# pangsu0613/TransCAR

Hardware: AMD Instinct MI355X
Metric: nuScenes frames/sec (6-cam+radar, 900 queries): fusion decoder (Detr3DHead.forward + box decode), FPN features resident in HBM (higher is better)
Workload: dtype f32 (linear steps and attention core of the batched launches: f16x2 split operands, 3 v_mfma_f32_16x16x32_f16 products, fp32 accumulate; activations of the 32-row tiles held as two f16 planes; 4- / 8-row tiles: f32 MFMA)

## Files before the change

transcar_amd/csrc/chain.hip:

```cpp
#include <stdlib.h>
#include <string.h>

#include <type_traits>

#include "kernels.hpp"
#ifdef TC_CHAIN_STAMPS
__device__ long long g_cam_stamps[4][8];
#define CAM_STAMP(slot)                                                                        \
  do {                                                                                         \
    if (blockIdx.x == 100 && (threadIdx.x & 63) == 0)                                          \
      g_cam_stamps[(threadIdx.x >> 6) & 3][(slot)] = __builtin_amdgcn_s_memtime();             \
  } while (0)
#endif
#include "rowdev.hpp"
#define TC_ONCE_LD(p) ldg4_stream(p)
#ifdef TC_CHAIN_DUMP
__device__ float* g_chain_dump;
__device__ long long g_chain_dump_floats;
#endif

namespace tc {

namespace {

// ... 7 lines not shown

struct StepRes {
  const float* p0; const float* p1; const float* p2; const float* p3;
  float* gd; float* gt;
  int K, N, gld, gmod;
  short kind, src, src2, dst, res, act, flags, sync, rep, si;
  int src_off, src2_off;
  int pad_;
};
struct EpiRec {
  float* gd; float* gt;
  int dst_off, res_off, dst_ld, res_ld;
  int gld, act, flags, N;
  int has_bias, woff;
  int drop_site;
  int pad1;
};
struct PreRec { const float* first; int nidx; int pad; };
template <int NW> struct StepAllT { StepRes r; EpiRec e; PreRec p[NW]; };
using StepAll = StepAllT<CH_NW>;
static_assert(sizeof(StepAllT<CH_NW>) % 16 == 0 && sizeof(StepAllT<CH_NW_MAX>) % 16 == 0, "records are copied 16 bytes at a time");
template <int N, int NW = CH_NW> struct Recs { StepAllT<NW> s[N]; };

constexpr int HM_WORDS = 8;
static_assert(HM_WORDS * 8 <= LDL * 4 && (LDL * 4) % 8 == 0, "hit masks live in a row of the logit buffer");
template <int R, int NREC>
struct ChainLds {
  StepAllT<nw_of(R)> recs[NREC];
  float unit[4][R][LD2];
  float l[R][LDL];
  float box[R][12];
  float cen[R][4];
  int gate[R];
  int rowg[R];
};
static_assert(LD5 * 1 <= 2 * LD2, "the 512-wide tile must fit two units");

#ifdef TC_CHAIN_STAMPS
#define CHAIN_DBG(v) (v)
#else
#define CHAIN_DBG(v) 0
#endif

#define MFMA44(a, b, c, grp) __builtin_amdgcn_mfma_f32_4x4x1f32((a), (b), (c), 4, (grp), 0)

enum Buf : short { B_NONE = -1, B_A = 0 , B_X , B_U1, B_U2, B_U3, B_L };
enum Kind : short {
  K_END = 0, K_LOAD, K_LINEAR, K_LN, K_POSENC, K_SAMPLE, K_REFUPD, K_TOKENS, K_RADAR_ATTN, K_BOXADD, K_RADAR_GATE,
  K_NARROW,
  K_NOP,
  K_LOADG,
  K_MASKCOPY,
  K_LN_BWD,
  K_ATTN_BWD
};
enum NSpecial : short { N_LOGITS = -1, N_CODE = -2, N_CLS = -3 };
enum Flags : short {
  F_GATE = 1,
  F_SCALEQ = 2,
  F_WOFF = 4,
  F_LN_RELU = 8,
  F_SKIP_NONEXT = 16,
  F_WAVE1 = 32,
  F_NOT_W0 = 64,
  F_LN_XP = 128,
  F_IFHIT = 256,
  F_GPRE = 512,
  F_CMASK = 1024,
  F_CMASK_SCALE = 2048,
  F_CARRY = 4096,
  F_NOT_LAYER0 = 8192,
  F_PRESYNC = 16384
};
enum GSel : short {
  G_NONE = -1, G_HS = 0, G_QK, G_VT, G_INITREF, G_ATTN_O, G_XIN, G_POS, G_CLS, G_KV0, G_KV1, G_KV2,
  G_QF, G_RFEAT, G_COUNT
};

struct StepDesc {
  short kind, wp, wp2, K, N, src, src2, dst, res, act, flags, gsel, gtsel, sync;
};
constexpr StepDesc PROG_DECODER_T[] = {
    {K_LOAD, 0, 0, 0, 0, B_NONE, B_NONE, B_U1, B_NONE, 0, 0, G_ATTN_O, G_NONE, 0},
    {K_LOAD, 0, 0, 0, 0, B_NONE, B_NONE, B_X, B_NONE, 0, 0, G_XIN, G_NONE, 1},
    {K_LINEAR, 1, -1, 256, 256, B_U1, B_NONE, B_U2, B_X, 0, 0, G_NONE, G_NONE, 1},
    {K_LN, 2, -1, 0, 0, B_U2, B_NONE, B_X, B_U1, 0, F_LN_XP, G_NONE, G_NONE, 1},
    {K_LINEAR, 3, -1, 256, N_LOGITS, B_U1, B_NONE, B_L, B_NONE, 0, 0, G_NONE, G_NONE, 0},
    {K_POSENC, 5, 6, 0, 0, B_NONE, B_NONE, B_U2, B_NONE, 0, F_NOT_W0, G_NONE, G_NONE, 1},
    {K_SAMPLE, 0, 0, 0, 0, B_L, B_NONE, B_U3, B_NONE, 0, 0, G_NONE, G_NONE, 1},
    {K_LINEAR, 7, -1, 256, 256, B_U2, B_NONE, B_U1, B_NONE, 0, 0, G_NONE, G_NONE, 1},
    {K_LINEAR, 4, -1, 256, 256, B_U3, B_NONE, B_U2, B_X, 0, 0, G_NONE, G_NONE, 1},
    {K_LN, 9, 8, 0, 0, B_U2, B_U1, B_X, B_NONE, 0, 0, G_NONE, G_NONE, 1},
    {K_LINEAR, 10, -1, 256, 512, B_X, B_NONE, B_A, B_NONE, 1, 0, G_NONE, G_NONE, 1},
    {K_LINEAR, 11, -1, 512, 256, B_A, B_NONE, B_U3, B_X, 0, 0, G_NONE, G_NONE, 1},
    {K_LN, 12, -1, 0, 0, B_U3, B_NONE, B_X, B_U1, 0, F_LN_XP, G_HS, G_NONE, 1},
    {K_LINEAR, 13, -1, 256, 256, B_X, B_NONE, B_U2, B_NONE, 1, 0, G_NONE, G_NONE, 0},
    {K_LINEAR, 16, -1, 256, 512, B_U1, B_NONE, B_NONE, B_NONE, 0, F_SCALEQ | F_SKIP_NONEXT, G_QK, G_NONE, 0},
    {K_LINEAR, 16, -1, 256, 256, B_X, B_NONE, B_NONE, B_NONE, 0, F_WOFF | F_SKIP_NONEXT, G_NONE, G_VT, 1},
    {K_LINEAR, 14, -1, 256, 256, B_U2, B_NONE, B_U3, B_NONE, 1, 0, G_NONE, G_NONE, 0},
    {K_NARROW, 15, -1, 256, N_CODE, B_U3, B_U1, B_L, B_NONE, 0, F_PRESYNC, G_NONE, G_NONE, 1},
    {K_REFUPD, 0, 0, 0, 0, B_L, B_NONE, B_NONE, B_NONE, 0, 0, G_NONE, G_NONE, 0},
    {K_END, 0, 0, 0, 0, 0, 0, 0, 0, 0, 0, 0, 0, 0}};
constexpr StepDesc PROG_DECODER_L0_T[] = {
    {K_LOAD, 0, 0, 0, 0, B_NONE, B_NONE, B_U1, B_NONE, 0, 0, G_ATTN_O, G_NONE, 0},
    {K_LOAD, 0, 0, 0, 0, B_NONE, B_NONE, B_U2, B_NONE, 0, 0, G_KV1, G_NONE, 0},
    {K_LOAD, 0, 0, 0, 0, B_NONE, B_NONE, B_X, B_NONE, 0, 0, G_XIN, G_NONE, 1},
    {K_LINEAR, 3, -1, 256, N_LOGITS, B_U1, B_NONE, B_L, B_NONE, 0, 0, G_NONE, G_NONE, 0},
// ... 25 lines not shown
    {K_LOAD, 0, 0, 0, 0, B_NONE, B_NONE, B_U1, B_NONE, 0, 0, G_POS, G_NONE, 0},
    {K_LOAD, 0, 0, 0, 0, B_NONE, B_NONE, B_X, B_NONE, 0, 0, G_XIN, G_NONE, 1},
    {K_LINEAR, 0, -1, 256, 3, B_U1, B_NONE, B_NONE, B_NONE, 2, 0, G_INITREF, G_NONE, 0},
    {K_LINEAR, 16, -1, 256, 512, B_X, B_U1, B_NONE, B_NONE, 0, F_SCALEQ, G_QK, G_NONE, 0},
    {K_LINEAR, 16, -1, 256, 256, B_X, B_NONE, B_NONE, B_NONE, 0, F_WOFF, G_NONE, G_VT, 0},
    {K_END, 0, 0, 0, 0, 0, 0, 0, 0, 0, 0, 0, 0, 0}};
constexpr StepDesc PROG_RADAR_ENC_T[] = {
    {K_TOKENS, 0, 0, 0, 0, B_NONE, B_NONE, B_A, B_NONE, 0, 0, G_NONE, G_NONE, 1},
    {K_POSENC, 0, 1, 0, 0, B_A, B_NONE, B_U3, B_NONE, 0, 0, G_NONE, G_NONE, 0},
    {K_LINEAR, 4, -1, 36, 64, B_A, B_NONE, B_X, B_NONE, 1, 0, G_NONE, G_NONE, 1},
    {K_LINEAR, 2, -1, 256, 256, B_U3, B_NONE, B_U1, B_NONE, 0, 0, G_NONE, G_NONE, 0},
    {K_LINEAR, 5, -1, 64, 128, B_X, B_NONE, B_U2, B_NONE, 1, 0, G_NONE, G_NONE, 1},
    {K_LINEAR, 6, -1, 128, 256, B_U2, B_NONE, B_X, B_NONE, 1, 0, G_NONE, G_NONE, 1},
    {K_LN, 3, -1, 0, 0, B_U1, B_NONE, B_U2, B_X, 0, F_LN_RELU, G_NONE, G_NONE, 1},
    {K_LINEAR, 7, -1, 256, 512, B_U2, B_NONE, B_NONE, B_NONE, 0, 0, G_KV0, G_NONE, 0},
    {K_LINEAR, 8, -1, 256, 512, B_U2, B_NONE, B_NONE, B_NONE, 0, 0, G_KV1, G_NONE, 0},
    {K_LINEAR, 9, -1, 256, 512, B_U2, B_NONE, B_NONE, B_NONE, 0, 0, G_KV2, G_NONE, 0},
    {K_END, 0, 0, 0, 0, 0, 0, 0, 0, 0, 0, 0, 0, 0}};
constexpr StepDesc PROG_RADAR_ENC_A_T[] = {
    {K_TOKENS, 0, 0, 0, 0, B_NONE, B_NONE, B_A, B_NONE, 0, 0, G_NONE, G_NONE, 1},
    {K_POSENC, 0, 1, 0, 0, B_A, B_NONE, B_U3, B_NONE, 0, 0, G_NONE, G_NONE, 0},
    {K_LINEAR, 4, -1, 36, 64, B_A, B_NONE, B_X, B_NONE, 1, 0, G_NONE, G_NONE, 1},
    {K_LINEAR, 2, -1, 256, 256, B_U3, B_NONE, B_U1, B_NONE, 0, 0, G_NONE, G_NONE, 0},
    {K_LINEAR, 5, -1, 64, 128, B_X, B_NONE, B_U2, B_NONE, 1, 0, G_NONE, G_NONE, 1},
    {K_LINEAR, 6, -1, 128, 256, B_U2, B_NONE, B_X, B_NONE, 1, 0, G_NONE, G_NONE, 1},
    {K_LN, 3, -1, 0, 0, B_U1, B_NONE, B_U2, B_X, 0, F_LN_RELU, G_RFEAT, G_NONE, 1},
    {K_LINEAR, 7, -1, 256, 512, B_U2, B_NONE, B_NONE, B_NONE, 0, 0, G_KV0, G_NONE, 0},
    {K_END, 0, 0, 0, 0, 0, 0, 0, 0, 0, 0, 0, 0, 0}};
constexpr StepDesc PROG_RADAR_ENC_B_T[] = {
    {K_LOAD, 0, 0, 0, 0, B_NONE, B_NONE, B_X, B_NONE, 0, 0, G_RFEAT, G_NONE, 1},
    {K_LINEAR, 8, -1, 256, 512, B_X, B_NONE, B_NONE, B_NONE, 0, 0, G_KV1, G_NONE, 0},
    {K_LINEAR, 9, -1, 256, 512, B_X, B_NONE, B_NONE, B_NONE, 0, 0, G_KV2, G_NONE, 0},
    {K_END, 0, 0, 0, 0, 0, 0, 0, 0, 0, 0, 0, 0, 0}};
constexpr StepDesc PROG_RADAR_LAYER_T[] = {
    {K_RADAR_GATE, 0, 0, 0, 0, B_NONE, B_NONE, B_NONE, B_NONE, 0, 0, G_NONE, G_NONE, 1},
    {K_LINEAR, 0, -1, 256, 256, B_X, B_NONE, B_U1, B_NONE, 0, F_SCALEQ | F_IFHIT, G_NONE, G_NONE, 1},
    {K_RADAR_ATTN, 0, 0, 0, 0, B_U1, B_NONE, B_U2, B_NONE, 0, F_IFHIT, G_NONE, G_NONE, 1},
    {K_LINEAR, 1, -1, 256, 256, B_U2, B_NONE, B_U3, B_X, 0, F_GATE | F_IFHIT, G_NONE, G_NONE, 1},
    {K_LN, 2, -1, 0, 0, B_U3, B_NONE, B_X, B_NONE, 0, 0, G_NONE, G_NONE, 1},
    {K_LINEAR, 3, -1, 256, 512, B_X, B_NONE, B_A, B_NONE, 1, 0, G_NONE, G_NONE, 1},
    {K_LINEAR, 4, -1, 512, 256, B_A, B_NONE, B_U3, B_X, 0, 0, G_NONE, G_NONE, 1},
    {K_LN, 5, -1, 0, 0, B_U3, B_NONE, B_X, B_NONE, 0, 0, G_NONE, G_NONE, 1},
    {K_LINEAR, 6, -1, 256, 256, B_X, B_NONE, B_U1, B_NONE, 0, 0, G_NONE, G_NONE, 0},
    {K_LINEAR, 11, -1, 256, 256, B_X, B_NONE, B_U2, B_NONE, 1, 0, G_NONE, G_NONE, 1},
    {K_LN, 7, -1, 0, 0, B_U1, B_NONE, B_U1, B_NONE, 0, F_LN_RELU, G_NONE, G_NONE, 0},
    {K_LINEAR, 12, -1, 256, 256, B_U2, B_NONE, B_U3, B_NONE, 1, 0, G_NONE, G_NONE, 1},
    {K_LINEAR, 8, -1, 256, 256, B_U1, B_NONE, B_U2, B_NONE, 0, 0, G_NONE, G_NONE, 1},
    {K_LN, 9, -1, 0, 0, B_U2, B_NONE, B_U2, B_NONE, 0, F_LN_RELU, G_NONE, G_NONE, 0},
    {K_NARROW, 13, -1, 256, N_CODE, B_U3, B_U1, B_L, B_NONE, 0, F_PRESYNC, G_NONE, G_NONE, 0},
    {K_NARROW, 10, -1, 256, N_CLS, B_U2, B_U1, B_NONE, B_NONE, 0, F_PRESYNC, G_CLS, G_NONE, 1},
    {K_BOXADD, 0, 0, 0, 0, B_L, B_NONE, B_NONE, B_NONE, 0, 0, G_NONE, G_NONE, 1},
    {K_END, 0, 0, 0, 0, 0, 0, 0, 0, 0, 0, 0, 0, 0}};

constexpr StepDesc PROG_RADAR_BWD_T[] = {
    {K_LOADG, 0, 0, 0, N_CODE, B_NONE, B_NONE, B_U1, B_NONE, 0, F_CARRY, G_NONE, G_NONE, 1},
    {K_LINEAR, 13, -1, N_CODE, 256, B_U1, B_NONE, B_U2, B_NONE, 0, F_CMASK, G_NONE, G_NONE, 1},
    {K_LINEAR, 12, -1, 256, 256, B_U2, B_NONE, B_U1, B_NONE, 0, F_CMASK, G_NONE, G_NONE, 1},
    {K_LINEAR, 11, -1, 256, 256, B_U1, B_NONE, B_U3, B_X, 0, 0, G_NONE, G_NONE, 1},
    {K_LOADG, 0, 0, 0, N_CLS, B_NONE, B_NONE, B_U1, B_NONE, 0, 0, G_NONE, G_NONE, 1},
    {K_LINEAR, 10, -1, N_CLS, 256, B_U1, B_NONE, B_U2, B_NONE, 0, 0, G_NONE, G_NONE, 1},
    {K_LN_BWD, 9, -1, 0, 0, B_U2, B_NONE, B_U1, B_X, 0, F_LN_RELU, G_NONE, G_NONE, 1},
    {K_LINEAR, 8, -1, 256, 256, B_U1, B_NONE, B_U2, B_NONE, 0, 0, G_NONE, G_NONE, 1},
    {K_LN_BWD, 7, -1, 0, 0, B_U2, B_NONE, B_U1, B_X, 0, F_LN_RELU, G_NONE, G_NONE, 1},
    {K_LINEAR, 6, -1, 256, 256, B_U1, B_NONE, B_X, B_U3, 0, 0, G_NONE, G_NONE, 1},
    {K_LN_BWD, 5, -1, 0, 0, B_X, B_NONE, B_X, B_U1, 0, 0, G_NONE, G_NONE, 1},
    {K_MASKCOPY, 0, 0, 3, 0, B_X, B_NONE, B_U3, B_NONE, 0, 0, G_NONE, G_NONE, 1},
    {K_LINEAR, 4, -1, 256, 512, B_U3, B_NONE, B_A, B_NONE, 0, F_CMASK | F_CMASK_SCALE, G_NONE, G_NONE, 1},
    {K_LINEAR, 3, -1, 512, 256, B_A, B_NONE, B_U3, B_X, 0, 0, G_NONE, G_NONE, 1},
    {K_LN_BWD, 2, -1, 0, 0, B_U3, B_NONE, B_X, B_U1, 0, 0, G_NONE, G_NONE, 1},
    {K_MASKCOPY, 0, 0, 1, 0, B_X, B_NONE, B_U1, B_NONE, 0, F_GATE, G_NONE, G_NONE, 1},
    {K_LINEAR, 1, -1, 256, 256, B_U1, B_NONE, B_U2, B_NONE, 0, 0, G_NONE, G_NONE, 1},
    {K_ATTN_BWD, 0, 0, 0, 0, B_U2, B_NONE, B_U1, B_NONE, 0, 0, G_NONE, G_NONE, 1},
    {K_LINEAR, 0, -1, 256, 256, B_U1, B_NONE, B_X, B_X, 0, F_NOT_LAYER0, G_NONE, G_NONE, 1},
    {K_END, 0, 0, 0, 0, 0, 0, 0, 0, 0, 0, 0, 0, 0}};
enum DSel : short { D_NONE = -1, D_DBOX = 0, D_DT1, D_DT0, D_DC2, D_DC0, D_DFF, D_DH, D_DPROJ, D_DQP, D_DCLS, D_COUNT };
constexpr short BWD_STORE[19] = {D_DBOX, D_DT1, D_DT0, D_NONE, D_DCLS, D_NONE, D_DC2, D_NONE, D_DC0, D_NONE, D_NONE, D_DFF,
                                 D_DH, D_NONE, D_NONE, D_DPROJ, D_NONE, D_DQP, D_NONE};
enum Program : int { PROG_PROLOGUE = 0, PROG_DECODER, PROG_RADAR_ENC, PROG_RADAR, PROG_RADAR_ENC_A, PROG_RADAR_ENC_B,
                     PROG_RADAR_TRAIN, PROG_RADAR_ENC_TRAIN, PROG_RADAR_BWD };
constexpr bool prog_is_radar(int p) { return p == PROG_RADAR || p == PROG_RADAR_TRAIN; }
constexpr bool prog_is_enc_full(int p) { return p == PROG_RADAR_ENC || p == PROG_RADAR_ENC_TRAIN; }
enum TSel : short { T_NONE = -1, T_QP = 0, T_AO, T_X1, T_X2, T_H, T_FF, T_X3, T_C0, T_C1, T_C2, T_C3, T_T0, T_T1, T_TREG,
                    E_U0, E_U1, E_U2, E_POS, E_F0, E_F1, E_F2, E_MEM, T_COUNT };
constexpr short RADAR_TAPE[17] = {T_NONE, T_QP, T_AO, T_X1, T_X2, T_H, T_FF, T_X3, T_C0, T_T0, T_C1, T_T1, T_C2, T_C3,
                                  T_TREG, T_NONE, T_NONE};
constexpr short ENC_TAPE[10] = {T_NONE, E_U1, E_F0, E_U2, E_F1, E_F2, E_MEM, T_NONE, T_NONE, T_NONE};
constexpr short ENC_TAPE2[10] = {T_NONE, E_U0, T_NONE, T_NONE, T_NONE, T_NONE, E_POS, T_NONE, T_NONE, T_NONE};
constexpr short BWD_TAPE[19] = {T_NONE, T_T1, T_T0, T_NONE, T_NONE, T_NONE, T_C2, T_NONE, T_C0, T_NONE, T_X2, T_NONE,
                                T_H, T_NONE, T_X1, T_NONE, T_NONE, T_NONE, T_NONE};
constexpr short BWD_TAPE2[19] = {T_NONE, T_NONE, T_NONE, T_NONE, T_NONE, T_NONE, T_C3, T_NONE, T_C1, T_NONE, T_FF, T_NONE,
                                 T_NONE, T_NONE, T_NONE, T_NONE, T_NONE, T_NONE, T_NONE};

constexpr int MAX_PAIRS = 48;
constexpr int RADAR_PAIRS = 14;

struct ChainDev {
  int program, M, Q, code, ncls, nlogits, has_next, nlayers;
  int total, early_n;
  float* g[G_COUNT]; int g_ld[G_COUNT]; int g_mod[G_COUNT];
  float qscale; int qpad;
  DropK drop;
  int dbg;
  int tile_rows;
  int matrix_path;
  int last_cls_only;
  const float* ref_in; int ref_mod; float* ref_out; float* box_m;
// ... 1133 lines not shown
          if (row < R) act_st4<PL>(dst + row * LD2, 4 * lane, early_v[j][ri]);
        }
      }
    }
  }
#pragma unroll
  for (int t = 0; t < REC_TRIPS; ++t) {
    const int i = threadIdx.x + t * NT;
    if (i < REC16) reinterpret_cast<int4*>(&S.recs[0])[i] = rec_v[t];
  }
  START_STAMP(43);

  if (prog_is_radar(PROG)) {
    auto row_of = [&](int row) {
      const int pos = min(m0 + row, M - 1);
      return k.row_perm != nullptr ? k.row_perm[pos] : pos;
    };
    if (threadIdx.x < R) S.rowg[threadIdx.x] = row_of(threadIdx.x);
    for (int row = wave; row < R; row += NW) {
      const int grow = row_of(row);
      act_st4<PL>(&S.unit[0][row][0], 4 * lane, TC_ONCE_LD(k.g[G_QF] + (size_t)grow * 256 + 4 * lane));
    }
    {
      const int row = threadIdx.x >> 4, j = threadIdx.x & 15;
      if (row < R) {
        const int grow = row_of(row);
        if (j < k.code) S.box[row][j] = k.box_in[(size_t)grow * k.code + j];
        if (j >= 12 && j < 15) {
          const int c = j - 12;
          if (k.cen_from_box) {
            S.cen[row][c] = k.box_in[(size_t)grow * k.code + (c == 2 ? 4 : c)];
          } else {
            const float r = k.ref_last[(size_t)grow * 3 + c];
            const float* pc = k.cam.pc;
            S.cen[row][c] = c < 2 ? __fadd_rn(__fmul_rn(r, pc[3 + c] - pc[c]), pc[c]) : r;
          }
        }
      }
    }
  }
  if constexpr (PROG == PROG_RADAR_BWD) {
    for (int i = threadIdx.x; i < R * LD2; i += NT) (&S.unit[0][0][0])[i] = 0.0f;
    if (threadIdx.x < R * 12) (&S.box[0][0])[threadIdx.x] = 0.0f;
    if (threadIdx.x < R) S.gate[threadIdx.x] = 0;
  }
  __syncthreads();

  START_STAMP(46);
#ifdef TC_CHAIN_STAMPS
  int stamp_i = 0;
  STEP_STAMP();
#endif

  auto do_ln = [&](const StepRes& r) {
    constexpr int NR = R / NW;
    const float* a = buf_ptr(S, r.src); const int lda = buf_ld(r.src);
    const float* c = buf_ptr(S, r.src2); const int ldc = buf_ld(r.src2);
    const bool xp = (r.flags & F_LN_XP) != 0;
    const float* dd = xp ? nullptr : buf_ptr(S, r.res);
    float* dst2 = xp ? buf_ptr(S, r.res) : nullptr;
    float* dst = buf_ptr(S, r.dst);
    float* gdst = r.gd;
    float4 gg, bb;
    if (CHAIN_DBG(k.dbg) & (1 << 17)) {
      gg = make_float4(1.f, 1.f, 1.f, 1.f); bb = make_float4(0.f, 0.f, 0.f, 0.f);
    } else {
      gg = ld4(r.p0 + 4 * lane); bb = ld4(r.p1 + 4 * lane);
    }
    float4 v[NR], pos4[NR];
#pragma unroll
    for (int i = 0; i < NR; ++i) {
      const int row = wave + NW * i;
      pos4[i] = make_float4(0.f, 0.f, 0.f, 0.f);
      if (xp && !(CHAIN_DBG(k.dbg) & (1 << 18))) {
        int prow = min(m0 + row, M - 1);
        if (k.g_mod[G_POS] > 0) prow = prow % k.g_mod[G_POS];
        pos4[i] = ld4(k.g[G_POS] + (size_t)prow * k.g_ld[G_POS] + 4 * lane);
      }
      v[i] = act_ld4<PL>(a + row * lda, 4 * lane);
    }
    if (c != nullptr) {
      const float4 g2 = ld4(r.p2 + 4 * lane), b2 = ld4(r.p3 + 4 * lane);
      float4 cv[NR];
#pragma unroll
      for (int i = 0; i < NR; ++i) cv[i] = act_ld4<PL>(c + (wave + NW * i) * ldc, 4 * lane);
      ln_rows<NR>(cv, g2, b2);
#pragma unroll
      for (int i = 0; i < NR; ++i) v[i] = add4(v[i], relu4(cv[i]));
    }
    ln_rows<NR>(v, gg, bb);
#pragma unroll
    for (int i = 0; i < NR; ++i) {
      const int row = wave + NW * i;
      if (r.flags & F_LN_RELU) v[i] = relu4(v[i]);
      if constexpr (PROG == PROG_RADAR_ENC_TRAIN) {
        if (r.gt != nullptr && m0 + row < M) st4(r.gt + (size_t)(m0 + row) * 256 + 4 * lane, v[i]);
      }
      if (dd != nullptr) v[i] = add4(v[i], act_ld4<PL>(dd + row * LD2, 4 * lane));
      act_st4<PL>(dst + row * LD2, 4 * lane, v[i]);
      if (xp) act_st4<PL>(dst2 + row * LD2, 4 * lane, add4(v[i], pos4[i]));
      if (gdst != nullptr && m0 + row < M) st4(gdst + (size_t)(m0 + row) * 256 + 4 * lane, v[i]);
    }
  };
  auto lin_spec = [&](const StepRes& r) {
    LinSpec s;
    s.K = r.K; s.N = r.N;
    s.W = r.p0; s.bias = r.p1;
    const float* lbase = reinterpret_cast<const float*>(smem_raw);
    s.src = lbase + r.src_off; s.src_ld = buf_ld(r.src);
// ... 23 lines not shown
    s.act = e.act;
    s.scale = (e.flags & F_SCALEQ) ? k.qscale : 1.0f; s.scale_cols = (e.flags & F_SCALEQ) ? 256 : 0;
    s.gdst = e.gd; s.gdst_ld = e.gld;
    s.gt = (e.flags & F_CMASK) ? nullptr : e.gt; s.gt_ld = k.qpad; s.gt_rpb = k.Q;
    s.cmask = (e.flags & F_CMASK) ? e.gt : nullptr;
    s.cscale = (e.flags & F_CMASK_SCALE) ? k.rdrop.scale : 1.0f;
    s.m0 = m0; s.M = M;
    s.woff = e.woff;
    s.dbg = 0;
    s.sub_on = 0;
    s.drop_site = 0; s.drop_seed = 0; s.drop_thr = 0; s.drop_scale = 1.0f; s.drop_stride = 0; s.drop_q = 0;
    s.rowg = (prog_is_radar(PROG) && k.row_perm != nullptr) ? &S.rowg[0] : nullptr;
    s.gpre = (e.flags & F_GPRE) ? 1 : 0;
    s.dst_pl = PL && e.dst_ld != LDL; s.res_pl = PL && e.res_ld != LDL;
    s.range_flag = MM == 1 ? k.range_status : nullptr;
    if (DROP) {
      if constexpr (PROG == PROG_RADAR_TRAIN) {
        s.drop_site = e.drop_site; s.drop_seed = k.rdrop.seed; s.drop_thr = k.rdrop.thr; s.drop_scale = k.rdrop.scale;
      } else {
        s.drop_site = e.drop_site; s.drop_seed = k.drop.seed; s.drop_thr = k.drop.thr; s.drop_scale = k.drop.scale;
        s.drop_stride = k.drop.seed_stride; s.drop_q = (int)k.drop.rows_per_sample;
      }
    }
    return s;
  };

  auto tile_has_hit = [&]() {
    int any = 0;
#pragma unroll
    for (int i = 0; i < R; ++i) any |= S.gate[i];
    return __builtin_amdgcn_readfirstlane(any) > 0;
  };

#ifdef TC_CHAIN_DUMP
  auto dump_step = [&](int step, int dst_id) {
    if constexpr (PROG == PROG_RADAR) {
      __syncthreads();
      float* out = g_chain_dump;
      const float* src = buf_ptr(S, dst_id);
      if (out != nullptr && src != nullptr && dst_id != B_L && (long long)(step + 1) * M * 256 <= g_chain_dump_floats) {
        const int ld = buf_ld(dst_id);
        for (int row = wave; row < R; row += NW)
          if (m0 + row < M)
            st4(out + ((size_t)step * M + S.rowg[row]) * 256 + 4 * lane, *reinterpret_cast<const float4*>(src + row * ld + 4 * lane));
      }
      __syncthreads();
    }
  };
#define DUMP_STEP(step, dst) dump_step((step), (dst))
#else
#define DUMP_STEP(step, dst) do {} while (0)
#endif
  int idx = (CHAIN_DBG(k.dbg) & 16) ? total : early_n;
#ifdef TC_CHAIN_STAMPS
  for (int j = 0; j < 2 * early_n; ++j) STEP_STAMP();
#endif
#pragma unroll 1
  while (idx < total) {
    const int kind = ufirst(S.recs[idx].r.kind);
    if (kind == K_LINEAR || kind == K_LN || kind == K_NOP) {
      WBuf w0;
      int pre_idx = -1;
#ifdef TC_CHAIN_STAMPS
      int ln_rep = 0;
#endif
#pragma unroll 1
      for (;;) {
        const StepRes r = load_uniform<StepRes>(S.recs[idx].r);
        const int kd = r.kind;
        bool skip = false;
        if constexpr (PROG == PROG_RADAR) {
          if (kd == K_LINEAR && (r.flags & F_IFHIT)) skip = !tile_has_hit();
        }
        if (skip) {
          if (r.res != B_NONE && r.dst != B_NONE) {
            const float* rs = buf_ptr(S, r.res); const int rld = buf_ld(r.res);
            float* dd = buf_ptr(S, r.dst);
            for (int row = wave; row < R; row += NW)
              *reinterpret_cast<float4*>(dd + row * LD2 + 4 * lane) = *reinterpret_cast<const float4*>(rs + row * rld + 4 * lane);
          }
        } else if (kd == K_LINEAR) {
          LinSpec s = lin_spec(r);
#ifdef TC_CHAIN_STAMPS
          s.sub_on = (r.si == g_sub_step && r.rep == 0);
          SUB_STAMP(0);
#endif
          if (((wave - s.woff) & (NW - 1)) < (R == 32 ? (s.N + 31) >> 5 : (s.N + 63) >> 6)) {
            const PreRec pr = load_uniform<PreRec>(S.recs[idx].p[wave]);
            const bool have = linear_step<R, DROP, PROG == PROG_PROLOGUE, MM, MP>(s, w0, pre_idx == idx, pr.first, epi_spec, idx);
            pre_idx = have ? pr.nidx : -1;
          }
        } else if (kd == K_LN) {
          if (!(CHAIN_DBG(k.dbg) & 4)) do_ln(r);
#ifdef TC_CHAIN_STAMPS
          if (ln_rep < ((k.dbg >> 19) & 3)) { ++ln_rep; continue; }
          ln_rep = 0;
#endif
        } else if (kd != K_NOP) {
          break;
        }
        STEP_STAMP();
        if (r.sync && !(CHAIN_DBG(k.dbg) & 2)) __syncthreads();
        STEP_STAMP();
        DUMP_STEP(idx, r.dst);
        if (++idx >= total) break;
      }
      continue;
    }
    const StepRes r = load_uniform<StepRes>(S.recs[idx].r);
    const int rep = r.rep;
    switch (kind) {
      case K_LOAD: { if constexpr (PROG == PROG_DECODER || PROG == PROG_PROLOGUE || PROG == PROG_RADAR_ENC_B) {
        constexpr int MAXL = 3, RW = (R + NW - 1) / NW;
        int n = 1;
        while (n < MAXL && idx + n < total && ufirst(S.recs[idx + n].r.kind) == K_LOAD) ++n;
        float4 v[MAXL][RW];
        float* dsts[MAXL];
        int any_sync = 0;
#pragma unroll
        for (int j = 0; j < MAXL; ++j) {
          if (j < n) {
            const StepRes rj = load_uniform<StepRes>(S.recs[idx + j].r);
            const float* gsrc = rj.gd;
            const int ld = rj.gld, mod = rj.gmod;
            dsts[j] = buf_ptr(S, rj.dst);
            any_sync |= rj.sync;
#pragma unroll
            for (int ri = 0; ri < RW; ++ri) {
              int grow = min(m0 + wave + ri * NW, M - 1);
              if (mod > 0) grow = grow % mod;
              v[j][ri] = TC_ONCE_LD(gsrc + (size_t)grow * ld + 4 * lane);
            }
          }
        }
#pragma unroll
        for (int j = 0; j < MAXL; ++j) {
          if (j < n) {
#pragma unroll
            for (int ri = 0; ri < RW; ++ri) {
              const int row = wave + ri * NW;
              if (row < R) act_st4<PL>(dsts[j] + row * LD2, 4 * lane, v[j][ri]);
            }
          }
        }
        for (int j = 0; j < n; ++j) { STEP_STAMP(); STEP_STAMP(); }
        if (any_sync) __syncthreads();
        idx += n;
        continue;
      }
      } break;
      case K_TOKENS: { if constexpr (prog_is_enc_full(PROG) || PROG == PROG_RADAR_ENC_A) {
        if constexpr (PL) {
          for (int i = threadIdx.x; i < R * 16; i += NT) {
            const int row = i >> 4, c4 = 4 * (i & 15);
            const int grow = min(m0 + row, M - 1);
            const float* tk = k.tokens + (size_t)grow * k.RI;
            act_st4<PL>(&S.unit[1][0][0] + row * LD5, c4,
// ... 198 lines not shown
        const int N = r.N;
        const int c = lane & 15, g = lane >> 4;
        const int rgw = wave >> 2, kq = wave & 3;
        const float* Wn = uptr(r.p0) + (size_t)min(c, N - 1) * 256 + 4 * g;
        const float* src = buf_ptr(S, r.src) + min(16 * rgw + c, R - 1) * buf_ld(r.src);
        float4 av[4], bw[4];
#pragma unroll
        for (int q = 0; q < 4; ++q) bw[q] = ld4(Wn + 16 * (4 * kq + q));
        const float bias = r.p1 != nullptr ? ldg1(uptr(r.p1) + min(c, N - 1)) : 0.0f;
        if (r.flags & F_PRESYNC) __syncthreads();
#pragma unroll
        for (int q = 0; q < 4; ++q) av[q] = act_ld4<PL>(src, 4 * g + 16 * (4 * kq + q));
        f32x4 acc = {0.f, 0.f, 0.f, 0.f};
#pragma unroll
        for (int q = 0; q < 4; ++q) {
          acc = MFMA16(av[q].x, bw[q].x, acc); acc = MFMA16(av[q].y, bw[q].y, acc);
          acc = MFMA16(av[q].z, bw[q].z, acc); acc = MFMA16(av[q].w, bw[q].w, acc);
        }
        float* part = buf_ptr(S, r.src2);
#pragma unroll
        for (int i = 0; i < 4; ++i) part[(wave * 16 + 4 * g + i) * 16 + c] = acc[i];
        __syncthreads();
        if (kq == 0 && c < N) {
          float y[4];
#pragma unroll
          for (int i = 0; i < 4; ++i) {
            const int prow = 4 * g + i;
            float v = part[(wave * 16 + prow) * 16 + c];
#pragma unroll
            for (int w = 1; w < 4; ++w) v += part[((wave + w) * 16 + prow) * 16 + c];
            y[i] = v + bias;
          }
          if (r.dst != B_NONE) {
            float* dd = buf_ptr(S, r.dst) + c;
            const int dld = buf_ld(r.dst);
#pragma unroll
            for (int i = 0; i < 4; ++i)
              if (16 * rgw + 4 * g + i < R) dd[(16 * rgw + 4 * g + i) * dld] = y[i];
          }
          if (r.gd != nullptr) {
#pragma unroll
            for (int i = 0; i < 4; ++i) {
              const int row = 16 * rgw + 4 * g + i;
              if (row < R && m0 + row < M) {
                int grow = m0 + row;
                if constexpr (prog_is_radar(PROG)) grow = S.rowg[row];
                stg1(r.gd + (size_t)grow * r.gld + c, y[i]);
              }
            }
          }
        }
      } break;
      } break;
      case K_RADAR_GATE: { if constexpr (prog_is_radar(PROG)) {
        constexpr int GW = 4;
        const bool keep = k.T <= 64 * HM_WORDS, cached = k.T <= 64 * GW;
        const int b0 = S.rowg[wave] / k.Q;
        float ty0[GW], ty1[GW];
        if (cached) {
          const float* rxy = k.tokens + (size_t)b0 * k.T * k.RI;
#pragma unroll
          for (int w = 0; w < GW; ++w) {
            const int t = min(64 * w + lane, k.T - 1);
            ty0[w] = rxy[(size_t)t * k.RI]; ty1[w] = rxy[(size_t)t * k.RI + 1];
          }
        }
        if (threadIdx.x < R) {
          const int i = threadIdx.x;
          const GateGeom::Pre pp = GateGeom::precompute(S.box[i][3], S.box[i][6], S.box[i][7], k.rmin[rep], k.rmax[rep]);
          S.box[i][10] = pp.ox; S.box[i][11] = pp.oy; S.cen[i][3] = pp.tstar;
        }
        __syncthreads();
#pragma unroll 1
        for (int row = wave; row < R; row += NW) {
          const int grow = S.rowg[row];
          const int b = grow / k.Q;
          int count = 0;
          if (cached && b == b0) {
            const GateGeom gg(S.cen[row][0], S.cen[row][1], GateGeom::Pre{S.box[row][10], S.box[row][11], S.cen[row][3]});
#pragma unroll
            for (int w = 0; w < GW; ++w) {
              if (64 * w < k.T) {
                const unsigned long long mask =
                    __ballot(64 * w + lane < k.T && gg.hit(ty0[w], ty1[w], sqnorm2(ty0[w], ty1[w])));
                count += __popcll(mask);
                if (k.T - 1 >= 64 * w && k.T - 1 < 64 * w + 64 && ((mask >> (k.T - 1 - 64 * w)) & 1ull)) count += k.pad_mult - 1;
                if (lane == 0) reinterpret_cast<unsigned long long*>(&S.l[row][0])[w] = mask;
              }
            }
          } else {
            count = radar_gate_count(S.cen[row][0], S.cen[row][1], S.box[row][3], S.box[row][6], S.box[row][7],
                                     k.rmin[rep], k.rmax[rep], k.tokens + (size_t)b * k.T * k.RI, k.RI, k.T,
                                     k.pad_mult, lane, keep ? reinterpret_cast<unsigned long long*>(&S.l[row][0]) : nullptr);
          }
          if (lane == 0) {
            S.gate[row] = count;
            if (m0 + row < M) k.hits[(size_t)rep * (k.hits_stride ? k.hits_stride : (size_t)M) + grow] = count;
          }
        }
      } break;
      } break;
      case K_RADAR_ATTN: { if constexpr (prog_is_radar(PROG)) {
        if (PROG == PROG_RADAR && (r.flags & F_IFHIT) && !tile_has_hit()) break;
#pragma unroll 1
        for (int row = wave; row < R; row += NW) {
          const int grow = S.rowg[row];
          const int b = grow / k.Q;
          float4 q4 = act_ld4<PL>(buf_ptr(S, r.src) + row * LD2, 4 * lane);
          const float* kv = (rep == 0 ? k.g[G_KV0] : rep == 1 ? k.g[G_KV1] : k.g[G_KV2]);
          int count = 0;
          const GateGeom gg(S.cen[row][0], S.cen[row][1], GateGeom::Pre{S.box[row][10], S.box[row][11], S.cen[row][3]});
          const unsigned long long* hm = k.T <= 64 * HM_WORDS ? reinterpret_cast<const unsigned long long*>(&S.l[row][0]) : nullptr;
          float4 o;
          if constexpr (PROG == PROG_RADAR_TRAIN) {
            q4.x *= k.qscale; q4.y *= k.qscale; q4.z *= k.qscale; q4.w *= k.qscale;
            DropK dk = k.rdrop;
            dk.site = 4u * (unsigned)rep;
            o = radar_attn_row_g<true>(gg, q4, k.tokens + (size_t)b * k.T * k.RI, k.RI, kv + (size_t)b * k.T * 512, 512,
                                       k.T, k.pad_mult, lane, count, dk, grow, hm);
            if (m0 + row < M) st4(r.gd + (size_t)grow * 256 + 4 * lane, o);
          } else {
            o = radar_attn_row_g(gg, q4, k.tokens + (size_t)b * k.T * k.RI, k.RI, kv + (size_t)b * k.T * 512, 512,
                                 k.T, k.pad_mult, lane, count, DropK(), 0, hm);
          }
          act_st4<PL>(buf_ptr(S, r.dst) + row * LD2, 4 * lane, o);
          if (lane == 0) S.gate[row] = count;
        }
      } break;
      } break;
      case K_LOADG: { if constexpr (PROG == PROG_RADAR_BWD) {
        const int N = r.N;
        float* dst = buf_ptr(S, r.dst);
        const float* src = uptr(r.p0);
        const bool carry = (r.flags & F_CARRY) != 0;
        for (int i = threadIdx.x; i < R * 64; i += NT) {
          const int row = i >> 6, c = i & 63;
          const int grow = min(m0 + row, M - 1);
          float v = c < N ? ldg1(src + (size_t)grow * N + c) : 0.0f;
          if (k.loss_vals != nullptr) {
            const float lv = k.loss_vals[2 * (k.nlayers - 1 - rep) + (carry ? 1 : 0)];
            if (!(fabsf(lv) <= 3.0e38f) || !(fabsf(v) <= 3.0e38f)) v = 0.0f;
          }
          if (carry && c < N) v += S.box[row][c];
          if (c < N && r.gd != nullptr && m0 + row < M) stg1(r.gd + (size_t)grow * N + c, v);
          dst[row * LD2 + c] = v;
        }
        if (carry) {
          __syncthreads();
          const int layer = k.nlayers - 1 - rep;
          if (blockIdx.x == 0 && threadIdx.x < 2 && k.loss_vals != nullptr && k.loss_out != nullptr) {
            const float lv = k.loss_vals[2 * layer + threadIdx.x];
            k.loss_out[2 * layer + threadIdx.x] = lv != lv ? 0.0f : lv;
          }
          if (threadIdx.x < R * 16) {
            const int row = threadIdx.x >> 4, c = threadIdx.x & 15;
            if (c < 12) S.box[row][c] = (c == 0 || c == 1 || c == 4) ? dst[row * LD2 + c] : 0.0f;
// ... 74 lines not shown
#pragma unroll
            for (int w = 1; w < NW; ++w) t += scratch[w * 256 + threadIdx.x];
            if (k.detp != nullptr) acc_add(*k.detp, gdst + threadIdx.x, t);
            else unsafeAtomicAdd(gdst + threadIdx.x, t);
          }
        }
      } break;
      } break;
      case K_ATTN_BWD: { if constexpr (PROG == PROG_RADAR_BWD) {
        const int layer = k.nlayers - 1 - rep;
        const float* dao = buf_ptr(S, r.src);
        float* dqb = buf_ptr(S, r.dst);
        DropK dk = k.rdrop;
        dk.site = 4u * (unsigned)layer;
        for (int row = wave; row < R; row += NW) {
          const int grow = min(m0 + row, M - 1);
          const int b = grow / k.Q;
          float4 dq = make_float4(0.f, 0.f, 0.f, 0.f);
          if (S.gate[row] > 0 && m0 + row < M) {
            const float* cxy = k.bwd_cxy[layer] + (size_t)grow * k.bwd_ldc[layer];
            const float* bx = k.bwd_box[layer] + (size_t)grow * k.code;
            float4 q4 = ld4(uptr(r.p0) + (size_t)grow * 256 + 4 * lane);
            q4.x *= k.qscale; q4.y *= k.qscale; q4.z *= k.qscale; q4.w *= k.qscale;
            const float4 o4 = ld4(uptr(r.p1) + (size_t)grow * 256 + 4 * lane);
            const float4 dO = *reinterpret_cast<const float4*>(dao + row * LD2 + 4 * lane);
            dq = radar_attn_bwd_row(cxy[0], cxy[1], bx[3], bx[6], bx[7], k.rmin[layer], k.rmax[layer], q4,
                                    k.tokens + (size_t)b * k.T * k.RI, k.RI, uptr(r.p2) + (size_t)b * k.T * 512,
                                    const_cast<float*>(uptr(r.p3)) + (size_t)b * k.T * 512, 512, k.T, k.pad_mult, dO, o4,
                                    dk, grow, lane,
                                    k.detp != nullptr ? det_shadow_of(*k.detp, uptr(r.p3) + (size_t)b * k.T * 512) : nullptr);
            dq.x *= k.qscale; dq.y *= k.qscale; dq.z *= k.qscale; dq.w *= k.qscale;
          }
          *reinterpret_cast<float4*>(dqb + row * LD2 + 4 * lane) = dq;
          if (r.gd != nullptr && m0 + row < M) st4(r.gd + (size_t)grow * 256 + 4 * lane, dq);
        }
      } break;
      } break;
      case K_BOXADD: { if constexpr (prog_is_radar(PROG)) {
        const int row = threadIdx.x >> 4, j = threadIdx.x & 15;
        if (row < R && j < k.code) {
          const int c = j == 0 ? 0 : j == 1 ? 1 : j == 4 ? 2 : -1;
          float bx = S.l[row][j];
          if (c >= 0) { bx += S.cen[row][c]; S.cen[row][c] = bx; }
          S.box[row][j] = bx;
          if (m0 + row < M) k.all_box[((size_t)rep * M + S.rowg[row]) * k.code + j] = bx;
        }
      } break;
      } break;
      default: break;
    }
    STEP_STAMP();
    if (r.sync) __syncthreads();
    STEP_STAMP();
    DUMP_STEP(idx, r.dst);
    ++idx;
  }
  WG_STAMP(1);
}

template <int R, int PROG, bool DROP = false, int MM = 0, bool PRE = false, bool MP = false>
__global__ __launch_bounds__(nw_of(R) * 64, 2) void chain_kernel(ChainDev k, Recs<rec_cap(PROG), nw_of(R)> recs) {
  chain_body<R, PROG, DROP, MM, PRE, MP>(k, recs.s, blockIdx.x);
}

template <int RA, int RB, int PROGB, int MM = 0, bool PRE = false, bool MP = false>
__global__ __launch_bounds__(nw_of(RA) * 64, 2) void chain_dual_kernel(ChainDev ka, ChainDev kb, int na,
                                                           Recs<rec_cap(PROG_DECODER), nw_of(RA)> ra,
                                                           Recs<rec_cap(PROGB), nw_of(RB)> rb) {
  static_assert(nw_of(RA) == nw_of(RB), "both programs of a launch run with the same workgroup size");
  if ((int)blockIdx.x < na) chain_body<RA, PROG_DECODER, false, MM, PRE, MP>(ka, ra.s, blockIdx.x);
  else chain_body<RB, PROGB, false, MM>(kb, rb.s, (int)blockIdx.x - na);
}

template <int R, int PROG>
int lds_off(int id) {
  using Lds = ChainLds<R, rec_cap(PROG)>;
  const int unit0 = (int)(offsetof(Lds, unit) / 4), ustride = R * LD2;
  switch (id) {
    case B_A: return unit0 + ustride;
    case B_X: return unit0;
    case B_U1: return unit0 + ustride;
    case B_U2: return unit0 + 2 * ustride;
    case B_U3: return unit0 + 3 * ustride;
    case B_L: return (int)(offsetof(Lds, l) / 4);
    default: return -1;
  }
}
template <int R, int PROG>
constexpr size_t chain_lds_bytes() { return sizeof(ChainLds<R, rec_cap(PROG)>); }
inline int buf_ld_h(int id) { return id == B_A ? LD5 : id == B_L ? LDL : LD2; }

template <int R, int PROG, int MM = 0>
void resolve_program(ChainK& k, StepAllT<nw_of(R)>* out) {
  constexpr int NW = nw_of(R);
  const StepDesc* table = prog_table(PROG);
  int nsteps = table_steps(PROG);
  if (PROG == PROG_DECODER && k.l0_seq != 0) {
    table = k.l0_seq == 1 ? PROG_DECODER_L0_T : PROG_DECODER_L0GEN_T;
    nsteps = (int)((k.l0_seq == 1 ? sizeof(PROG_DECODER_L0_T) : sizeof(PROG_DECODER_L0GEN_T)) / sizeof(StepDesc)) - 1;
  }
  const int nrep = (prog_is_radar(PROG) || PROG == PROG_RADAR_BWD) ? k.nlayers : 1;
  const int total = nsteps * nrep;
  memset(out, 0, sizeof(StepAllT<NW>) * rec_cap(PROG));
  for (int idx = 0; idx < total; ++idx) {
    const int rep = idx / nsteps, si = idx - rep * nsteps;
    const int layer = PROG == PROG_RADAR_BWD ? k.nlayers - 1 - rep : rep;
    const int pair0 = (prog_is_radar(PROG) || PROG == PROG_RADAR_BWD) ? layer * RADAR_PAIRS : 0;
    const StepDesc d = table[si];
    StepRes& r = out[idx].r;
    r.K = d.K; r.N = d.N;
    r.kind = d.kind; r.src = d.src; r.src2 = d.src2; r.dst = d.dst; r.res = d.res; r.act = d.act;
    r.flags = d.flags; r.sync = d.sync; r.rep = (short)rep; r.si = (short)si;
    if ((d.flags & F_SKIP_NONEXT) && !k.has_next) r.kind = K_NOP;
    if (PROG == PROG_DECODER && !k.refine &&
        (d.kind == K_REFUPD || ((d.kind == K_LINEAR || d.kind == K_NARROW) && d.wp >= 13 && d.wp <= 15)))
      r.kind = K_NOP;
    if (PROG == PROG_RADAR && k.last_cls_only && rep + 1 < nrep && d.wp >= 6 && d.wp <= 10 &&
        (d.kind == K_LINEAR || d.kind == K_LN || d.kind == K_NARROW))
      r.kind = K_NOP;
    if (d.gsel != G_NONE) { r.gd = k.g[d.gsel]; r.gld = k.g_ld[d.gsel]; r.gmod = k.g_mod[d.gsel]; }
    if (d.gtsel != G_NONE) r.gt = k.g[d.gtsel];
    bool taped = false;
    if (PROG == PROG_RADAR_TRAIN) {
      if (d.flags & F_SCALEQ) r.flags = (short)(r.flags & ~F_SCALEQ);
      r.flags = (short)(r.flags & ~F_IFHIT);
      if (d.kind == K_LINEAR && d.wp == 4) r.flags = (short)(r.flags | F_GPRE);
      const short ts = RADAR_TAPE[si];
      if (ts != T_NONE && r.gd == nullptr) { r.gd = k.tape[ts] + (size_t)rep * k.tape_stride; r.gld = 256; taped = true; }
    }
    if (PROG == PROG_RADAR_BWD) {
      if ((d.flags & F_NOT_LAYER0) && layer == 0) r.kind = K_NOP;
      const short ds = BWD_STORE[si], ts = BWD_TAPE[si], ts2 = BWD_TAPE2[si];
      if (ds != D_NONE && k.dy[ds] != nullptr) { r.gd = k.dy[ds] + (size_t)layer * k.dy_stride; taped = true; }
      const float* t1 = ts != T_NONE ? k.tape[ts] + (size_t)layer * k.tape_stride : nullptr;
      const float* t2 = ts2 != T_NONE ? k.tape[ts2] + (size_t)layer * k.tape_stride : nullptr;
      if (d.kind == K_LINEAR && (d.flags & F_CMASK)) r.gt = const_cast<float*>(t1);
      if (d.kind == K_LN_BWD) {
        const tc_linear n = k.pairs[pair0 + d.wp], gn = k.gpairs[pair0 + d.wp];
        r.p0 = n.w; r.p1 = t1; r.p2 = t2; r.gt = const_cast<float*>(gn.w); r.p3 = gn.b;
      }
      if (d.kind == K_LOADG) {
        r.N = d.N == N_CODE ? k.code : k.ncls;
        r.p0 = (d.N == N_CODE ? k.d_box : k.d_cls) + (size_t)layer * k.M * r.N;
      }
      if (d.kind == K_MASKCOPY) r.K = d.K;
      if (d.kind == K_ATTN_BWD) {
        r.p0 = k.tape[T_QP] + (size_t)layer * k.tape_stride; r.p1 = k.tape[T_AO] + (size_t)layer * k.tape_stride;
        r.p2 = k.g[G_KV0 + layer]; r.p3 = k.dkv[layer];
      }
    }
    if (PROG == PROG_RADAR_ENC_TRAIN) {
      const short ts = ENC_TAPE[si], ts2 = ENC_TAPE2[si];
      if (ts != T_NONE && r.gd == nullptr) { r.gd = k.tape[ts]; r.gld = 256; taped = true; }
      if (ts2 != T_NONE) r.gt = k.tape[ts2];
    }
    if (PROG == PROG_DECODER && d.N == N_LOGITS && generic_xattn(k)) r.dst = B_U3;
    if (d.kind == K_LINEAR) {
      const tc_linear pr = k.pairs[pair0 + d.wp];
      r.K = d.K == 36 ? k.RI : d.K == N_CODE ? k.code : d.K == N_CLS ? k.ncls : d.K;
      r.N = d.N == N_LOGITS ? k.nlogits : d.N == N_CODE ? k.code : d.N == N_CLS ? k.ncls : d.N;
      const int woff = (d.flags & F_WOFF) ? 512 : 0;
      r.p0 = pr.w + (size_t)woff * ((r.K + 63) & ~63);
      if (R >= 16) r.p0 += (MM == 1 ? 2 : 1) * k.w16_delta;
      r.p1 = pr.b ? pr.b + woff : nullptr;
      if (PROG == PROG_RADAR_BWD) r.p1 = nullptr;
      if (d.gsel == G_CLS) r.gd += (size_t)rep * k.M * k.ncls;
      if (taped) r.gld = r.N;
    } else if (d.kind == K_NARROW) {
      const tc_linear pr = k.pairs[pair0 + d.wp];
      r.N = d.N == N_CODE ? k.code : d.N == N_CLS ? k.ncls : d.N;
      r.p0 = pr.w; r.p1 = pr.b;
      if (d.gsel == G_CLS) r.gd += (size_t)rep * k.M * k.ncls;
      if (taped) r.gld = r.N;
    } else if (d.kind == K_LN || d.kind == K_POSENC) {
      const tc_linear n = k.pairs[pair0 + d.wp];
      r.p0 = n.w; r.p1 = n.b;
      if (d.kind == K_POSENC || d.src2 != B_NONE) {
        const tc_linear n2 = k.pairs[pair0 + d.wp2];
        r.p2 = n2.w; r.p3 = n2.b;
      }
    }
    r.src_off = lds_off<R, PROG>(r.src); r.src2_off = lds_off<R, PROG>(r.src2);
    EpiRec& e = out[idx].e;
    e.gd = r.gd; e.gt = r.gt; e.gld = r.gld; e.act = r.act; e.flags = r.flags; e.N = r.N;
    e.has_bias = r.p1 != nullptr; e.woff = (r.flags & F_WAVE1) ? 1 : 0;
    e.drop_site = 0;
    if (PROG == PROG_DECODER && k.drop.thr != 0 && d.kind == K_LINEAR) {
      const int off = d.wp == 1 ? 1 : d.wp == 4 ? 2 : d.wp == 10 ? 3 : d.wp == 11 ? 4 : 0;
      if (off) e.drop_site = (int)k.drop.site + off + 1;
    }
    if (PROG == PROG_RADAR_TRAIN && d.kind == K_LINEAR) {
      const int off = d.wp == 1 ? 1 : d.wp == 3 ? 2 : d.wp == 4 ? 3 : 0;
      if (off) e.drop_site = 4 * rep + off + 1;
    }
    e.dst_off = lds_off<R, PROG>(r.dst); e.dst_ld = buf_ld_h(r.dst);
    e.res_off = lds_off<R, PROG>(r.res); e.res_ld = buf_ld_h(r.res);
  }
  for (int idx = 0; idx < total; ++idx) {
    for (int w = 0; w < NW; ++w) {
      PreRec& pr = out[idx].p[w];
      pr.first = nullptr; pr.nidx = -1;
      for (int j = idx + 1; j < total; ++j) {
        const StepRes& n = out[j].r;
        if (n.kind == K_LN || n.kind == K_NOP) continue;
        if (n.kind != K_LINEAR) break;
        const int vw = (w - ((n.flags & F_WAVE1) ? 1 : 0)) & (NW - 1);
        const size_t kpad = (size_t)((n.K + 63) & ~63);
        if (R == 32) {
          if (vw >= ((n.N + 31) >> 5)) continue;
          pr.nidx = j;
          pr.first = n.p0 + (size_t)(vw >> 1) * 64 * kpad + (size_t)(vw & 1) * 4 * 256;
        } else {
          if (vw >= ((n.N + 63) >> 6)) continue;
          pr.nidx = j;
          pr.first = n.p0 + (size_t)vw * 64 * kpad;
        }
        break;
      }
    }
  }
// ... 518 lines not shown
```

Measured before the change: 10440.

## Fuse radar reg/cls heads and box add into one MFMA step; skip gated steps by jump

For the 32-row radar program, the separate reg and cls narrow projections and the box-add step are replaced by a single K_HEADS step. Waves split across heads and K-quarters, use 16x16 MFMA with partial sums reduced in LDS, and then write box and class outputs directly. Tiles with no radar hit now jump past the gated linear/attention steps in one go and point the following LayerNorm at the residual buffer. Previously each skipped step was evaluated and the residual was copied into place. This removes per-step dispatch, syncs and the copy, but adds new code paths that could diverge numerically or in correctness.

```diff
diff --git a/transcar_amd/csrc/chain.hip b/transcar_amd/csrc/chain.hip
--- a/transcar_amd/csrc/chain.hip
+++ b/transcar_amd/csrc/chain.hip
@@ -83,7 +83,8 @@
   K_LOADG,
   K_MASKCOPY,
   K_LN_BWD,
-  K_ATTN_BWD
+  K_ATTN_BWD,
+  K_HEADS
 };
 enum NSpecial : short { N_LOGITS = -1, N_CODE = -2, N_CLS = -3 };
 enum Flags : short {
@@ -215,6 +216,23 @@
     {K_BOXADD, 0, 0, 0, 0, B_L, B_NONE, B_NONE, B_NONE, 0, 0, G_NONE, G_NONE, 1},
     {K_END, 0, 0, 0, 0, 0, 0, 0, 0, 0, 0, 0, 0, 0}};
 
+constexpr int radar_gate_skip() {
+  int n = 0;
+  while (PROG_RADAR_LAYER_T[1 + n].flags & F_IFHIT) ++n;
+  return n;
+}
+static_assert(radar_gate_skip() > 0 && PROG_RADAR_LAYER_T[0].kind == K_RADAR_GATE && PROG_RADAR_LAYER_T[0].sync &&
+                  PROG_RADAR_LAYER_T[radar_gate_skip()].kind == K_LINEAR && PROG_RADAR_LAYER_T[radar_gate_skip()].res != B_NONE &&
+                  PROG_RADAR_LAYER_T[radar_gate_skip() + 1].kind == K_LN &&
+                  PROG_RADAR_LAYER_T[radar_gate_skip() + 1].src == PROG_RADAR_LAYER_T[radar_gate_skip()].dst,
+              "a hit-free tile continues at the LayerNorm behind the gated steps");
+constexpr int RADAR_HEADS_SI = (int)(sizeof(PROG_RADAR_LAYER_T) / sizeof(StepDesc)) - 4;
+static_assert(PROG_RADAR_LAYER_T[RADAR_HEADS_SI].kind == K_NARROW && PROG_RADAR_LAYER_T[RADAR_HEADS_SI].N == N_CODE &&
+                  PROG_RADAR_LAYER_T[RADAR_HEADS_SI + 1].kind == K_NARROW && PROG_RADAR_LAYER_T[RADAR_HEADS_SI + 1].N == N_CLS &&
+                  PROG_RADAR_LAYER_T[RADAR_HEADS_SI + 2].kind == K_BOXADD &&
+                  PROG_RADAR_LAYER_T[RADAR_HEADS_SI].src2 == PROG_RADAR_LAYER_T[RADAR_HEADS_SI + 1].src2,
+              "K_HEADS stands for reg.4, cls.6 and the box add");
+
 constexpr StepDesc PROG_RADAR_BWD_T[] = {
     {K_LOADG, 0, 0, 0, N_CODE, B_NONE, B_NONE, B_U1, B_NONE, 0, F_CARRY, G_NONE, G_NONE, 1},
     {K_LINEAR, 13, -1, N_CODE, 256, B_U1, B_NONE, B_U2, B_NONE, 0, F_CMASK, G_NONE, G_NONE, 1},
@@ -1454,9 +1472,9 @@
   STEP_STAMP();
 #endif
 
-  auto do_ln = [&](const StepRes& r) {
+  auto do_ln = [&](const StepRes& r, int src_id) {
     constexpr int NR = R / NW;
-    const float* a = buf_ptr(S, r.src); const int lda = buf_ld(r.src);
+    const float* a = buf_ptr(S, src_id); const int lda = buf_ld(src_id);
     const float* c = buf_ptr(S, r.src2); const int ldc = buf_ld(r.src2);
     const bool xp = (r.flags & F_LN_XP) != 0;
     const float* dd = xp ? nullptr : buf_ptr(S, r.res);
@@ -1586,6 +1604,7 @@
 #define DUMP_STEP(step, dst) do {} while (0)
 #endif
   int idx = (CHAIN_DBG(k.dbg) & 16) ? total : early_n;
+  int ln_src = B_NONE;
 #ifdef TC_CHAIN_STAMPS
   for (int j = 0; j < 2 * early_n; ++j) STEP_STAMP();
 #endif
@@ -1602,18 +1621,7 @@
       for (;;) {
         const StepRes r = load_uniform<StepRes>(S.recs[idx].r);
         const int kd = r.kind;
-        bool skip = false;
-        if constexpr (PROG == PROG_RADAR) {
-          if (kd == K_LINEAR && (r.flags & F_IFHIT)) skip = !tile_has_hit();
-        }
-        if (skip) {
-          if (r.res != B_NONE && r.dst != B_NONE) {
-            const float* rs = buf_ptr(S, r.res); const int rld = buf_ld(r.res);
-            float* dd = buf_ptr(S, r.dst);
-            for (int row = wave; row < R; row += NW)
-              *reinterpret_cast<float4*>(dd + row * LD2 + 4 * lane) = *reinterpret_cast<const float4*>(rs + row * rld + 4 * lane);
-          }
-        } else if (kd == K_LINEAR) {
+        if (kd == K_LINEAR) {
           LinSpec s = lin_spec(r);
 #ifdef TC_CHAIN_STAMPS
           s.sub_on = (r.si == g_sub_step && r.rep == 0);
@@ -1625,18 +1633,19 @@
             pre_idx = have ? pr.nidx : -1;
           }
         } else if (kd == K_LN) {
-          if (!(CHAIN_DBG(k.dbg) & 4)) do_ln(r);
+          if (!(CHAIN_DBG(k.dbg) & 4)) do_ln(r, (PROG == PROG_RADAR && ln_src != B_NONE) ? ln_src : (int)r.src);
 #ifdef TC_CHAIN_STAMPS
           if (ln_rep < ((k.dbg >> 19) & 3)) { ++ln_rep; continue; }
           ln_rep = 0;
 #endif
+          ln_src = B_NONE;
         } else if (kd != K_NOP) {
           break;
         }
         STEP_STAMP();
         if (r.sync && !(CHAIN_DBG(k.dbg) & 2)) __syncthreads();
         STEP_STAMP();
-        DUMP_STEP(idx, r.dst);
+        DUMP_STEP(r.rep * table_steps(PROG) + r.si, r.dst);
         if (++idx >= total) break;
       }
       continue;
@@ -1941,6 +1950,73 @@
         }
       } break;
       } break;
+      case K_HEADS: { if constexpr (PROG == PROG_RADAR && R == 32) {
+        const int c = lane & 15, g = lane >> 4;
+        const int hd = wave >> 2, kq = wave & 3;
+        const float* Wp = hd == 0 ? r.p0 : r.p2;
+        const float* bp = hd == 0 ? r.p1 : r.p3;
+        const bool on = Wp != nullptr;
+        const int N = hd == 0 ? k.code : k.ncls;
+        float4 bw[4];
+        float bias = 0.0f;
+        if (on) {
+          const float* Wn = uptr(Wp) + (size_t)min(c, N - 1) * 256 + 4 * g;
+#pragma unroll
+          for (int q = 0; q < 4; ++q) bw[q] = ld4(Wn + 16 * (4 * kq + q));
+          if (bp != nullptr) bias = ldg1(uptr(bp) + min(c, N - 1));
+        }
+        __syncthreads();
+        float* part = buf_ptr(S, r.src2);
+        if (on) {
+          const float* src = buf_ptr(S, hd == 0 ? r.src : r.res) + c * LD2;
+#pragma unroll 1
+          for (int rg = 0; rg < 2; ++rg) {
+            float4 av[4];
+#pragma unroll
+            for (int q = 0; q < 4; ++q) av[q] = act_ld4<PL>(src + 16 * rg * LD2, 4 * g + 16 * (4 * kq + q));
+            f32x4 acc = {0.f, 0.f, 0.f, 0.f};
+#pragma unroll
+            for (int q = 0; q < 4; ++q) {
+              acc = MFMA16(av[q].x, bw[q].x, acc); acc = MFMA16(av[q].y, bw[q].y, acc);
+              acc = MFMA16(av[q].z, bw[q].z, acc); acc = MFMA16(av[q].w, bw[q].w, acc);
+            }
+#pragma unroll
+            for (int i = 0; i < 4; ++i) part[(((hd * 2 + rg) * 4 + kq) * 16 + 4 * g + i) * 16 + c] = acc[i];
+          }
+        }
+        __syncthreads();
+        if (on && kq < 2 && c < N) {
+          const int rg = kq;
+          const float* pt = part + (hd * 2 + rg) * 4 * 256;
+          float y[4];
+#pragma unroll
+          for (int i = 0; i < 4; ++i) {
+            const int prow = 4 * g + i;
+            float v = pt[prow * 16 + c];
+#pragma unroll
+            for (int w = 1; w < 4; ++w) v += pt[(w * 16 + prow) * 16 + c];
+            y[i] = v + bias;
+          }
+          if (hd == 0) {
+            const int cc = c == 0 ? 0 : c == 1 ? 1 : c == 4 ? 2 : -1;
+#pragma unroll
+            for (int i = 0; i < 4; ++i) {
+              const int row = 16 * rg + 4 * g + i;
+              float bx = y[i];
+              if (cc >= 0) { bx += S.cen[row][cc]; S.cen[row][cc] = bx; }
+              S.box[row][c] = bx;
+              if (m0 + row < M) k.all_box[((size_t)rep * M + S.rowg[row]) * k.code + c] = bx;
+            }
+          } else {
+#pragma unroll
+            for (int i = 0; i < 4; ++i) {
+              const int row = 16 * rg + 4 * g + i;
+              if (m0 + row < M) stg1(r.gd + (size_t)S.rowg[row] * r.gld + c, y[i]);
+            }
+          }
+        }
+      } break;
+      } break;
       case K_RADAR_GATE: { if constexpr (prog_is_radar(PROG)) {
         constexpr int GW = 4;
         const bool keep = k.T <= 64 * HM_WORDS, cached = k.T <= 64 * GW;
@@ -1990,7 +2066,6 @@
       } break;
       } break;
       case K_RADAR_ATTN: { if constexpr (prog_is_radar(PROG)) {
-        if (PROG == PROG_RADAR && (r.flags & F_IFHIT) && !tile_has_hit()) break;
 #pragma unroll 1
         for (int row = wave; row < R; row += NW) {
           const int grow = S.rowg[row];
@@ -2171,8 +2246,17 @@
     STEP_STAMP();
     if (r.sync) __syncthreads();
     STEP_STAMP();
-    DUMP_STEP(idx, r.dst);
+    DUMP_STEP(r.rep * table_steps(PROG) + r.si, r.dst);
     ++idx;
+    if constexpr (PROG == PROG_RADAR) {
+      if (kind == K_RADAR_GATE && r.K > 0 && !tile_has_hit()) {
+        idx += r.K;
+        ln_src = r.N;
+#ifdef TC_CHAIN_STAMPS
+        for (int j = 0; j < 2 * r.K; ++j) STEP_STAMP();
+#endif
+      }
+    }
   }
   WG_STAMP(1);
 }
@@ -2219,10 +2303,13 @@
     nsteps = (int)((k.l0_seq == 1 ? sizeof(PROG_DECODER_L0_T) : sizeof(PROG_DECODER_L0GEN_T)) / sizeof(StepDesc)) - 1;
   }
   const int nrep = (prog_is_radar(PROG) || PROG == PROG_RADAR_BWD) ? k.nlayers : 1;
-  const int total = nsteps * nrep;
+  constexpr bool HEADS = PROG == PROG_RADAR && R == 32;
+  int total = 0;
   memset(out, 0, sizeof(StepAllT<NW>) * rec_cap(PROG));
-  for (int idx = 0; idx < total; ++idx) {
-    const int rep = idx / nsteps, si = idx - rep * nsteps;
+  for (int tidx = 0; tidx < nsteps * nrep; ++tidx) {
+    const int rep = tidx / nsteps, si = tidx - rep * nsteps;
+    if (HEADS && si > RADAR_HEADS_SI) continue;
+    const int idx = total++;
     const int layer = PROG == PROG_RADAR_BWD ? k.nlayers - 1 - rep : rep;
     const int pair0 = (prog_is_radar(PROG) || PROG == PROG_RADAR_BWD) ? layer * RADAR_PAIRS : 0;
     const StepDesc d = table[si];
@@ -2239,6 +2326,19 @@
       r.kind = K_NOP;
     if (d.gsel != G_NONE) { r.gd = k.g[d.gsel]; r.gld = k.g_ld[d.gsel]; r.gmod = k.g_mod[d.gsel]; }
     if (d.gtsel != G_NONE) r.gt = k.g[d.gtsel];
+    if (PROG == PROG_RADAR && d.kind == K_RADAR_GATE) {
+      r.K = radar_gate_skip(); r.N = table[radar_gate_skip()].res;
+    }
+    if (HEADS && si == RADAR_HEADS_SI) {
+      const StepDesc dc = table[si + 1], db = table[si + 2];
+      const tc_linear reg = k.pairs[pair0 + d.wp], cls = k.pairs[pair0 + dc.wp];
+      const bool has_cls = !(k.last_cls_only && rep + 1 < nrep);
+      r.kind = K_HEADS; r.flags = 0; r.sync = db.sync;
+      r.p0 = reg.w; r.p1 = reg.b;
+      r.p2 = has_cls ? cls.w : nullptr; r.p3 = has_cls ? cls.b : nullptr;
+      r.res = dc.src; r.dst = B_NONE;
+      r.gd = k.g[dc.gsel] + (size_t)rep * k.M * k.ncls; r.gld = k.g_ld[dc.gsel]; r.gmod = k.g_mod[dc.gsel];
+    }
     bool taped = false;
     if (PROG == PROG_RADAR_TRAIN) {
       if (d.flags & F_SCALEQ) r.flags = (short)(r.flags & ~F_SCALEQ);
@@ -2285,6 +2385,7 @@
       if (PROG == PROG_RADAR_BWD) r.p1 = nullptr;
       if (d.gsel == G_CLS) r.gd += (size_t)rep * k.M * k.ncls;
       if (taped) r.gld = r.N;
+    } else if (r.kind == K_HEADS) {
     } else if (d.kind == K_NARROW) {
       const tc_linear pr = k.pairs[pair0 + d.wp];
       r.N = d.N == N_CODE ? k.code : d.N == N_CLS ? k.ncls : d.N;
```

Result: slower. 10290 (-1.4%).
